# tungphambasement/DCNN

Hardware: AMD Instinct MI355X
Metric: images/sec (whole node) ResNet-18 Tiny-ImageNet training at 1/2/4/8 MI355X (higher is better)
Workload: dtype bf16; 1 GPU; model=resnet18_tiny_imagenet, global_batch=256, per_gpu_batch=256, parallelism=dp1, optimizer=adam, hipgraph=True, engine=native (C++ host API)

## Files before the change

### dcnn_amd/csrc/host/dcnn/ops.hpp

```cpp
#pragma once
#include <cstdint>

namespace dcnn {

struct ConvShape {
  int N, C, H, W, Co, KH, KW, SH, SW, PH, PW, OH, OW;
};
struct PoolShape {
  int N, C, H, W, OH, OW, KH, KW, SH, SW, PH, PW;
};
enum ActKind { ACT_RELU = 0, ACT_LEAKY_RELU = 1, ACT_ELU = 2, ACT_SIGMOID = 3, ACT_TANH = 4, ACT_LINEAR = 5 };

namespace cpu_ops {
void conv_fwd(const float* x, const float* w, const float* b, float* y, const ConvShape& s);
void conv_bwd(const float* x, const float* w, const float* dy, float* dx, float* dw, float* db, const ConvShape& s);
void dwconv_fwd(const float* x, const float* w, const float* b, float* y, const ConvShape& s);
void dwconv_bwd(const float* x, const float* w, const float* dy, float* dx, float* dw, float* db, const ConvShape& s);
void gconv_fwd(const float* x, const float* w, const float* b, float* y, const ConvShape& s, int groups);
void gconv_bwd(const float* x, const float* w, const float* dy, float* dx, float* dw, float* db, const ConvShape& s,
               int groups);
void dense_fwd(const float* x, const float* w, const float* b, float* y, long N, long In, long Out);
void dense_bwd(const float* x, const float* w, const float* dy, float* dx, float* dw, float* db, long N, long In,
               long Out);
void bn_fwd(const float* x, float* y, long N, long C, long HW, const float* g, const float* b, float eps, bool train,
// ... 14 lines not shown
void groupnorm_bwd(const float* x, const float* dy, const float* mean, const float* istd, const float* g, float* dx,
                   float* dg, float* db, long N, long C, long HW, long G);
void softmax_fwd(const float* x, float* y, long N, long C, long HW);
void softmax_bwd(const float* y, const float* dy, float* dx, long N, long C, long HW);
void dropout(const float* x, float* y, long n, float p, uint64_t seed);
void add(const float* a, const float* b, float* y, long n, bool relu);
void relu_mask(const float* dy, const float* y, float* dx, long n);
void adam(float* p, const float* g, float* m, float* v, long n, float lr, float b1, float b2, float eps, float bc1,
          float bc2, float wd, bool decoupled);
void sgd(float* p, const float* g, float* vel, long n, float lr, float momentum);
}

namespace gpu_ops {
void begin_deferred_reduce();
void end_deferred_reduce();
void flush_deferred_reduce();
void set_fault(int f);
void input_to_nhwc(const float* x, void* y, int N, int C, int HW);
void nhwc_to_nchw(const void* x, void* y, int N, int HW, int C);
void nchw_to_nhwc_bf16(const void* x, void* y, int N, int HW, int C);
void cast_bf16(const float* x, void* y, long n);
void zero(void* p, long nbytes);
const float* conv_fwd(const void* x, const void* w, const float* bias, void* y, const ConvShape& s,
                      int* stat_rows = nullptr);
struct BnbOperands {
  const void* y;
  const void* x;
  const float* mean;
  const float* istd;
  const float* gamma = nullptr;
  const float* beta = nullptr;
  bool mask_from_x = false;
};
const float* conv_dgrad(const void* dy, const void* w, void* dx, const ConvShape& s, const void* residual = nullptr,
                        bool w_transposed = false, const BnbOperands* bnb = nullptr, int* bnb_rows = nullptr);
void weight_transpose(const void* w, void* wt, int Co, int T, int C);
void multi_weight_transpose(const int64_t* table, int n, long max_tiles);
void conv_wgrad(const void* dy, const void* x, float* gw, float* gb, const ConvShape& s);
void dwconv_fwd(const void* x, const void* w, const float* bias, void* y, const ConvShape& s);
void dwconv_dgrad(const void* dy, const void* w, void* dx, const ConvShape& s, const void* residual = nullptr);
void dwconv_wgrad(const void* dy, const void* x, float* gw, float* gb, const ConvShape& s);
void gconv_fwd(const void* x, const void* w, const float* bias, void* y, const ConvShape& s, int groups);
void gconv_dgrad(const void* dy, const void* w, void* dx, const ConvShape& s, int groups,
                 const void* residual = nullptr);
void gconv_wgrad(const void* dy, const void* x, float* gw, float* gb, const ConvShape& s, int groups);
bool stem_ok(const ConvShape& s);
const float* stem_fwd(const float* x, const void* w, const float* bias, void* y, const ConvShape& s,
                      int* stat_rows = nullptr);
void stem_wgrad(const void* dy, const float* x, float* gw, float* gb, const ConvShape& s);
struct StemBn {
  const void* x;
  const float* mean;
  const float* istd;
// ... 93 lines not shown
```

### dcnn_amd/csrc/host/dist.cpp

```cpp
#include "dcnn/dist.hpp"

#include <arpa/inet.h>
#include <netdb.h>
#include <netinet/in.h>
#include <netinet/tcp.h>
#include <poll.h>
#include <sys/socket.h>
#include <unistd.h>

#include <cerrno>
#include <chrono>
#include <cstdlib>
#include <cstring>
#include <stdexcept>
#include <thread>

#include <algorithm>
#include <cstdint>

#include "../kernels/collective.h"
#include "dcnn/nn.hpp"
#include "dcnn/ops.hpp"

namespace dcnn {
// ... 414 lines not shown
    }
    if (!flow_) flow_ = gpu::flow_create();
    if (!ev_) ev_ = gpu::event_create();
  }
  reduced_lo_ = n_;
  next_ = lo_.size();
  nb_ = 0;
  model.set_backward_hook([this](size_t i) { on_layer_done(i); });
}

void DataParallel::reduce_layers(size_t lo_layer, size_t hi_layer) {
  if (comm_) {
    size_t lo = SIZE_MAX;
    for (size_t j = lo_layer; j < hi_layer; ++j) lo = std::min(lo, lo_[j]);
    if (lo == SIZE_MAX || lo >= reduced_lo_) return;
    gpu_ops::flush_deferred_reduce();
    gpu::event_record(ev_);
    gpu::flow_wait(flow_, ev_);
    comm_->all_reduce(g_ + lo, g_ + lo, reduced_lo_ - lo, 0, 4, flow_);
    reduced_lo_ = lo;
    ++nb_;
    return;
  }
  size_t total = 0;
  for (size_t j = lo_layer; j < hi_layer; ++j) total += layer_elems_[j];
  if (total == 0) return;
  pack_.resize(total);
  size_t o = 0;
  for (size_t j = lo_layer; j < hi_layer; ++j)
    for (const auto& s : segs_[j]) {
      std::memcpy(pack_.data() + o, s.first, s.second * 4);
// ... 2 lines not shown
  all_reduce_mean(pack_.data(), total);
  o = 0;
  for (size_t j = lo_layer; j < hi_layer; ++j)
    for (const auto& s : segs_[j]) {
      std::memcpy(s.first, pack_.data() + o, s.second * 4);
      o += s.second;
    }
  ++nb_;
}

void DataParallel::on_layer_done(size_t layer) {
  if (lo_.empty() || layer >= next_) return;
  size_t pending = 0;
  for (size_t j = layer; j < next_; ++j) pending += layer_elems_[j];
  if (pending == 0 || pending < bucket_elems_) return;
  reduce_layers(layer, next_);
  next_ = layer;
}

void DataParallel::finish() {
  if (lo_.empty()) throw std::runtime_error("DataParallel::finish: attach() first");
  if (next_ > 0) reduce_layers(0, next_);
  if (comm_) {
    gpu::event_record(ev_, flow_);
    gpu::flow_wait(gpu::flow(), ev_);
  }
  nb_last_ = nb_;
  nb_ = 0;
  reduced_lo_ = n_;
  next_ = lo_.size();
}

P2PLink::P2PLink(const std::string& unique_id, int rank, bool sender, int device) : sender_(sender) {
  if (!coll::available()) throw std::runtime_error("dist: RCCL unavailable: " + coll::load_error());
  if (rank != 0 && rank != 1) throw std::invalid_argument("P2PLink: rank 0 or 1");
  gpu::set_device(device);
  peer_ = 1 - rank;
// ... 92 lines not shown
```

### dcnn_amd/csrc/host/nn.cpp

```cpp
#include "dcnn/nn.hpp"

#include "../kernels/fusion_plan.h"

#include <algorithm>
#include <chrono>
#include <cmath>
#include <cstdio>
#include <cstdlib>
#include <filesystem>
#include <fstream>
#include <iostream>
#include <sstream>
#include <stdexcept>

namespace dcnn {

namespace {
struct Rng {
  uint64_t s;
  explicit Rng(uint64_t seed) : s(seed * 0x9e3779b97f4a7c15ull + 0x632be59bd9b4e019ull) {}
  uint64_t next() {
    uint64_t z = (s += 0x9e3779b97f4a7c15ull);
    z = (z ^ (z >> 30)) * 0xbf58476d1ce4e5b9ull;
    z = (z ^ (z >> 27)) * 0x94d049bb133111ebull;
// ... 157 lines not shown
  const Tensor& x_ = mbc().a;
  const ConvShape s = shape_for(x_.shape());
  gpu_ops::stem_wgrad_bn(dy.data(), x_.ptr<float>(), params_[0].grad.ptr<float>(),
                         bias_ ? params_[1].grad.ptr<float>() : nullptr, s, bn);
}

Tensor Conv2D::backward(const Tensor& dy) {
  const Tensor& x_ = mbc().a;
  const ConvShape s = shape_for(x_.shape());
  float* gb = bias_ ? params_[1].grad.ptr<float>() : nullptr;
  if (dev_.is_gpu() && x_.dtype() == DType::F32) {
    gpu_ops::stem_wgrad(dy.data(), x_.ptr<float>(), params_[0].grad.ptr<float>(), gb, s);
    return Tensor();
  }
  if (dev_.is_gpu()) {
    gpu_ops::conv_wgrad(dy.data(), x_.data(), params_[0].grad.ptr<float>(), gb, s);
    if (!input_grad_) return Tensor();
    Tensor dx = act_empty(x_.shape(), dev_);
    bool tr = false;
    const void* w = dgrad_operand(tr);
    if (bnb_from_ != nullptr) {
      const gpu_ops::BnbOperands ops = bnb_from_->bnb_operands(mb_);
      int rows = 0;
      const float* st = gpu_ops::conv_dgrad(dy.data(), w, dx.data(), s, nullptr, tr, &ops, &rows);
      if (rows > 0) bnb_from_->offer_bwd_stats(dx.data(), st, rows);
      return dx;
    }
    gpu_ops::conv_dgrad(dy.data(), w, dx.data(), s, nullptr, tr);
    return dx;
  }
  Tensor dx = act_empty(x_.shape(), dev_);
  {
    cpu_ops::conv_bwd(x_.ptr<float>(), params_[0].value.ptr<float>(), dy.ptr<float>(), dx.ptr<float>(),
                      params_[0].grad.ptr<float>(), gb, s);
  }
  return dx;
}

Tensor Conv2D::backward_residual(const Tensor& dy, const Tensor& residual) {
  const Tensor& x_ = mbc().a;
  if (!dev_.is_gpu() || x_.dtype() == DType::F32 || residual.shape() != x_.shape())
    throw std::runtime_error(name_ + ": backward_residual is a GPU fusion");
  const ConvShape s = shape_for(x_.shape());
  float* gb = bias_ ? params_[1].grad.ptr<float>() : nullptr;
  gpu_ops::conv_wgrad(dy.data(), x_.data(), params_[0].grad.ptr<float>(), gb, s);
  Tensor dx = act_empty(x_.shape(), dev_);
  bool tr = false;
  const void* w = dgrad_operand(tr);
  if (bnb_block_from_ != nullptr) {
    const gpu_ops::BnbOperands ops = bnb_block_from_->bnb_operands(mb_);
    int rows = 0;
    const float* st = gpu_ops::conv_dgrad(dy.data(), w, dx.data(), s, residual.data(), tr, &ops, &rows);
    if (rows > 0) bnb_block_from_->offer_bwd_stats(dx.data(), st, rows);
    return dx;
  }
  gpu_ops::conv_dgrad(dy.data(), w, dx.data(), s, residual.data(), tr);
  return dx;
}

DepthwiseConv2D::DepthwiseConv2D(int channels, int kh, int kw, int sh, int sw, int ph, int pw, bool bias,
// ... 1825 lines not shown
```

### dcnn_amd/csrc/host/ops_gpu.hip

```cpp
#include <hip/hip_runtime.h>

#include <algorithm>
#include <cmath>
#include <cstdio>
#include <cstdlib>
#include <cstring>
#include <map>
#include <mutex>
#include <stdexcept>
#include <string>
#include <unordered_map>
#include <vector>

#include "../kernels/api.h"
#include "dcnn/ops.hpp"
#include "dcnn/tensor.hpp"

#define HOST_HIP_CHECK(x)                                                                    \
  do {                                                                                       \
    hipError_t e_ = (x);                                                                     \
    if (e_ != hipSuccess) throw std::runtime_error(std::string(#x) + ": " + hipGetErrorString(e_)); \
  } while (0)

namespace dcnn {
// ... 444 lines not shown

void wgrad_reduce(const Tensor& hold, const Tensor& bhold, const float* slab, float* gw, long n, const float* bslab,
                  float* gb, long nb, int splits) {
  if (g_defer) {
    g_pending.push_back({hold, gw, n, splits});
    if (gb) g_pending.push_back({bhold, gb, nb, splits});
    g_pending_bytes += (size_t)n * splits * 4 + (gb ? (size_t)nb * splits * 4 : 0);
    if (reduce_flush_bytes() && g_pending_bytes >= reduce_flush_bytes()) launch_pending();
    return;
  }
  if (gb)
    splitk_reduce2(slab, gw, n, bslab, gb, nb, splits, 1, cur());
  else
    splitk_reduce(slab, gw, n, splits, 1, cur());
}
}

void begin_deferred_reduce() { g_defer = true; }
void set_fault(int f) { g_fault = f; }
void flush_deferred_reduce() {
  const bool on = g_defer;
  end_deferred_reduce();
  g_defer = on;
}
void end_deferred_reduce() {
  launch_pending();
  g_defer = false;
}

namespace {
void launch_pending() {
  for (size_t b = 0; b < g_pending.size(); b += kMaxRed) {
    MultiRed t{};
    t.count = (int)std::min(g_pending.size() - b, (size_t)kMaxRed);
    for (int k = 0; k < t.count; ++k) {
      const PendingRed& e = g_pending[b + k];
      t.e[k].slab = e.slab.ptr<float>();
      t.e[k].out = e.out;
      t.e[k].n = e.n;
      t.e[k].splits = e.splits;
    }
    multi_splitk_reduce(t, cur());
  }
  g_pending.clear();
  g_pending_bytes = 0;
}
// ... 164 lines not shown
      if (bnb && all_taps) {
        a.bnb = ba;
        a.stats = slab_of(gemm_g2_stat_rows(a.M, s.C));
      }
      gemm_g2(a, cur());
      return a.stats;
    }
  }
  NtArgs a{static_cast<const bf16*>(dy), wt, dx, s.N * s.H * s.W, s.C, K, 0, K, s.C, kConvDgrad, s.N, s.OH, s.OW,
           s.Co, s.H, s.W, s.KH, s.KW, s.SH, s.SW, s.PH, s.PW, nullptr, static_cast<const bf16*>(residual), nullptr,
           0, 0};
  gemm_nt(a, cur());
  return nullptr;
}

void conv_wgrad(const void* dy, const void* x, float* gw, float* gb, const ConvShape& s) {
  const int Ng = s.KH * s.KW * s.C, P = s.N * s.OH * s.OW;
  const long dyb = (long)P * s.Co * 2, xb = (long)s.N * s.H * s.W * s.C * 2;
  const int route = conv_wgrad_route(route_geom(s, -1));
  rec("wgrad", s, route, {{"bias", gb != nullptr}, {"deferred", g_defer}});
  if (route == ROUTE_HALO) {
    const int splits = hwgrad_splits(s.N, s.H, s.W, s.C, s.Co);
    Tensor hold, bhold;
    float* slab = wgrad_slab(SLAB, (size_t)splits * s.Co * Ng * 4, hold);
    float* bslab = gb ? wgrad_slab(BSLAB, (size_t)splits * s.Co * 4, bhold) : nullptr;
    HWArgs a{};
    a.dY = static_cast<const bf16*>(dy); a.X = static_cast<const bf16*>(x); a.slab = slab; a.bias_slab = bslab;
    a.dy_bytes = (unsigned)dyb; a.x_bytes = (unsigned)xb;
    a.NB = s.N; a.H = s.H; a.W = s.W; a.Cs = s.C; a.Co = s.Co; a.ntaps = 9;
    for (int t = 0; t < 9; ++t) { a.tap_dy[t] = t / 3 - 1; a.tap_dx[t] = t % 3 - 1; }
// ... 431 lines not shown
```

### dcnn_amd/csrc/kernels/api.h

```cpp
#pragma once
#include <hip/hip_runtime.h>
#include <stdint.h>

#include "fusion_plan.h"
typedef __bf16 bf16;

namespace dcnn {
struct BnbArgs {
  const bf16* y; const bf16* x; const float* mean; const float* istd;
  const float* gamma; const float* beta; int mask_x;
};
struct NtArgs {
  const bf16* A; const bf16* B; void* C;
  int M, N, K; int lda, ldb, ldc; int mode;
  int nb, sh, sw, cs, gh, gw; int kh, kw, strh, strw, padh, padw;
  const float* bias; const bf16* residual; float* stats; int out_f32; int relu;
};
struct TnArgs {
  const bf16* dY; const bf16* X; float* slab; float* bias_slab;
  int M, N, P; int mode; int nb, sh, sw, cs, gh, gw; int kh, kw, strh, strw, padh, padw; int ldx; int k_per_split;
};
struct G2Args {
  const bf16* A; const bf16* B; bf16* C;
  unsigned a_bytes, b_bytes;
// ... 63 lines not shown
void hconv3_enable(int on);
void hconv3_set_grid_cap(int n);
void hconv3_set_stamps(uintptr_t p);
struct HWArgs {
  const bf16* dY; const bf16* X; float* slab; float* bias_slab;
  unsigned dy_bytes, x_bytes;
  int NB, H, W, Cs, Co, ntaps;
  int tap_dy[9], tap_dx[9];
  int TH, TW, IMG, HPR, tiles_per_split;
  int ldy, ldx, npairs;
  int pair_yoff[3], pair_xoff[3], pair_bias[3];
};
void hwgrad(HWArgs a, int splits, hipStream_t s);
bool hwgrad_supported(int NB, int H, int W, int Cs, int Co, int ntaps);
int hwgrad_splits(int NB, int H, int W, int Cs, int Co);
bool hwgrad_f32_supported(int NB, int H, int W, int Cs, int Co);
int hwgrad_f32_splits(int NB, int H, int W, int Cs, int Co);
void hwgrad_f32(HWArgs a, int splits, hipStream_t s);
void hwgrad_set_version(int v);
bool hwgrad_s2_supported(int NB, int H, int W, int Cs, int Co);
int hwgrad_s2_splits(int NB, int H, int W, int Cs, int Co);
void hwgrad_s2(HWArgs a, int splits, hipStream_t s);

void gemm_nt(const NtArgs& a, hipStream_t s);
void gemm_g2(const G2Args& a, hipStream_t s);
void gemm_g2_set_splitk(int on);
int gemm_g2_splitk_enabled();
int gemm_g2_stat_rows(int M, int N);
int gemm_g2_row_tile(int M, int N);
void gemm_t2(T2Args a, int splits, hipStream_t s);
// ... 159 lines not shown
```

### dcnn_amd/csrc/kernels/bindings.cpp

```cpp
#include <tuple>
#include <pybind11/pybind11.h>
#include <pybind11/stl.h>
#include <algorithm>
#include <array>
#include <vector>
#include <hip/hip_runtime.h>
#include <stdint.h>

namespace py = pybind11;
#include "api.h"


using namespace dcnn;
void bind_runtime(py::module_& m);
void bind_rccl(py::module_& m);
template <typename T>
static inline T P(uintptr_t x) { return reinterpret_cast<T>(x); }
static inline hipStream_t S(uintptr_t x) { return reinterpret_cast<hipStream_t>(x); }

static void bind_gemm_g2(uintptr_t A, uintptr_t B, uintptr_t C, unsigned a_bytes, unsigned b_bytes, int M, int N, int Cs,
                         int H, int W, int GH, int GW, int SY, int SX, std::vector<std::array<int, 4>> taps, int ldb,
                         int ldc, int OH, int OW, int OSY, int OSX, int ORY, int ORX, uintptr_t bias, uintptr_t residual,
                         uintptr_t stats, int relu, uintptr_t zero_ptr, int zero_n, std::array<uintptr_t, 4> bnb,
                         uintptr_t stream, std::vector<std::array<int, 4>> classes = {}) {
// ... 129 lines not shown
          HWArgs a{};
          if (pairs.size() > 3) throw std::runtime_error("hwgrad: at most 3 operand pairs");
          a.npairs = (int)pairs.size(); a.ldy = ldy; a.ldx = ldx;
          for (size_t q = 0; q < pairs.size(); ++q) {
            a.pair_yoff[q] = pairs[q][0]; a.pair_xoff[q] = pairs[q][1]; a.pair_bias[q] = pairs[q][2];
          }
          a.dY = P<const bf16*>(dY); a.X = P<const bf16*>(X); a.slab = P<float*>(slab);
          a.bias_slab = P<float*>(bias_slab);
          a.dy_bytes = dy_bytes; a.x_bytes = x_bytes;
          a.NB = NB; a.H = H; a.W = W; a.Cs = Cs; a.Co = Co;
          if (taps.size() > 9 || taps.empty()) throw std::runtime_error("hwgrad: 1..9 taps");
          a.ntaps = (int)taps.size();
          for (size_t i = 0; i < taps.size(); ++i) { a.tap_dy[i] = taps[i][0]; a.tap_dx[i] = taps[i][1]; }
          hwgrad(a, splits, S(stream));
        });
  m.def("hwgrad_supported", &hwgrad_supported);
  m.def("hwgrad_s2_supported", &hwgrad_s2_supported);
  m.def("hwgrad_s2_splits", &hwgrad_s2_splits);
  m.def("hwgrad_s2",
        [](uintptr_t dY, uintptr_t X, uintptr_t slab, uintptr_t bias_slab, unsigned dy_bytes, unsigned x_bytes, int NB,
           int H, int W, int Cs, int Co, int splits, uintptr_t stream) {
          HWArgs a{};
          a.dY = P<const bf16*>(dY); a.X = P<const bf16*>(X); a.slab = P<float*>(slab);
          a.bias_slab = P<float*>(bias_slab);
          a.dy_bytes = dy_bytes; a.x_bytes = x_bytes;
          a.NB = NB; a.H = H; a.W = W; a.Cs = Cs; a.Co = Co; a.ntaps = 9;
          hwgrad_s2(a, splits, S(stream));
        });
  m.def("hwgrad_f32",
        [](uintptr_t dY, uintptr_t X, uintptr_t slab, uintptr_t bias_slab, unsigned dy_bytes, unsigned x_bytes, int NB,
// ... 447 lines not shown
```

### dcnn_amd/csrc/kernels/hwgrad.hip

```cpp
#include <type_traits>

#include "common.h"
#include "api.h"

namespace dcnn {

namespace {
constexpr unsigned kOOBw = 0x80000000u;
constexpr int PT = 128;

__device__ __forceinline__ void glds16w(i32x4 rsrc, char* lds, unsigned voff) { glds16_opaque(rsrc, lds, voff); }

__device__ __forceinline__ int xcd_remap_w(int bid, int nwg) {
  const int xcd = bid & 7, q = nwg >> 3, r = nwg & 7;
  const int base = xcd < r ? xcd * (q + 1) : r * (q + 1) + (xcd - r) * q;
  return base + (bid >> 3);
}

__device__ __forceinline__ int wswz(int row) { return (((row >> 1) & 1) | (((row >> 3) & 1) << 1)) << 1; }

__device__ __forceinline__ bf16x4 tr4(const char* base, int row, int col) {
  const int chn = col >> 3, within = (col & 7) * 2;
  const char* addr = base + row * 128 + ((chn ^ wswz(row)) << 4) + within;
  return __builtin_amdgcn_ds_read_tr16_b64_v4bf16((__attribute__((address_space(3))) bf16x4*)(const_cast<char*>(addr)));
// ... 204 lines not shown
  static_assert(TPX * IMG == PT, "tile must hold 128 pixels");
};

template <int K, int N, class F>
__device__ __forceinline__ void h3w_static_for(F&& f) {
  if constexpr (K < N) {
    f(std::integral_constant<int, K>{});
    h3w_static_for<K + 1, N>(f);
  }
}

__device__ __forceinline__ bf16x4 tr4_at(const char* addr) {
  return __builtin_amdgcn_ds_read_tr16_b64_v4bf16((__attribute__((address_space(3))) bf16x4*)(const_cast<char*>(addr)));
}

template <int TW, int TH, int IMG, int NS, int TSP = 1, bool F32 = false, bool C32 = false>
__global__ void __launch_bounds__(256 * TSP, 1) hwgrad2_kernel(HWArgs p) {
  prefetch_kernargs<sizeof(HWArgs)>();
  using G = HWGeo2<TW, TH, IMG>;
  constexpr int HNI = G::HNI, HW2P = G::HW2P, HPIP = G::HPIP, HPP = G::HPP, TPX = G::TPX, STAGE = G::STAGE;
  constexpr int INS = 4 + HNI;
  static_assert(NS == 2 || NS == 3, "2 or 3 stages");
  extern __shared__ __attribute__((aligned(16))) char smem[];
  const int tid = threadIdx.x, lane = tid & 63, wid = (tid >> 6) & 3, th = tid >> 8;
  constexpr int NT = 256 * TSP;
  const int co_tiles = p.Co / 64, ci_chunks = (p.Cs + 63) / 64;
  const int per_split = co_tiles * ci_chunks;
  const int lt = xcd_remap_w(blockIdx.x, gridDim.x);
  const int split = lt / per_split, rem = lt - split * per_split;
  const int pair = blockIdx.y, nsplits = gridDim.x / per_split;
  const int yoff = p.pair_yoff[pair], xoff = p.pair_xoff[pair];
  const int co0 = (rem / ci_chunks) * 64, c0 = (rem % ci_chunks) * 64;

  const int tx_tiles = p.W / TW, ty_tiles = p.H / TH, tpi = tx_tiles * ty_tiles;
  const int total_tiles = (p.NB / IMG) * tpi;
  const int tbeg = split * p.tiles_per_split;
  const int tend = min(total_tiles, tbeg + p.tiles_per_split);
  const i32x4 rsY = raw_rsrc(p.dY, p.dy_bytes);
  const i32x4 rsX = raw_rsrc(p.X, p.x_bytes);

  const int slot = lane & 7;
  unsigned y_rel[4], y_col[4];
#pragma unroll
  for (int i = 0; i < 4; ++i) {
    const int row = (wid * 4 + i) * 8 + (lane >> 3);
    const int im = row / TPX, r2 = row - im * TPX;
    y_rel[i] = (unsigned)((im * p.H + r2 / TW) * p.W + r2 % TW);
    y_col[i] = (unsigned)((yoff + co0 + ((slot ^ wswz2(row)) * 8)) * 2);
  }
  int h_rel[HNI], h_hy[HNI], h_hx[HNI];
#pragma unroll
  for (int j = 0; j < HNI; ++j) {
    const int row = (wid * HNI + j) * 8 + (lane >> 3);
    const int im = row / HPIP, r2 = row - im * HPIP;
// ... 63 lines not shown
        fb[k0][d] = PT * 128 + row * 128 + (((fci >> 2) ^ wswz2(row)) << 4) + (fci & 3) * 4;
      }
    }
  }
  auto blk_rows = [](int b) constexpr {
    if (TW == 16) return b * HW2P;
    if (TW == 8) return (b / 4) * HPIP + (b % 4) * 2 * HW2P;
    return b * HPIP;
  };

  auto run_f32 = [&](auto tb_c, auto ntw_c) {
    constexpr int TB = decltype(tb_c)::value, NTW = decltype(ntw_c)::value;
    f32x4 acc[NTW];
#pragma unroll
    for (int t = 0; t < NTW; ++t) acc[t] = f32x4{0.f, 0.f, 0.f, 0.f};
    const bool do_bias = p.bias_slab != nullptr && c0 == 0 && th == 0;
    float bias_acc = 0.f;
    if (NS == 3 && nt > 1)
      asm volatile("s_waitcnt vmcnt(%0)" ::"n"(INS) : "memory");
    else
      asm volatile("s_waitcnt vmcnt(0)" ::: "memory");
    __syncthreads();
    int cur = 0;
    for (int it = 0; it < nt; ++it) {
      if (it + NS - 1 < nt) load_tile(cur == 0 ? NS - 1 : cur - 1, tbeg + it + NS - 1);
      const char* S0 = smem + cur * STAGE;
      auto lds_f = [&](int off) { return *reinterpret_cast<const float*>(S0 + off); };
      float a[2], b[2][NTW];
      auto rd = [&](auto blk_c, int k0, int c) {
        constexpr int B = decltype(blk_c)::value;
        a[c] = lds_f(fa[k0] + B * 16 * 128);
// ... 17 lines not shown
      });
      if (do_bias) {
        const int col = tid & 31;
        for (int r = tid >> 5; r < PT; r += 8)
          bias_acc += *reinterpret_cast<const float*>(S0 + r * 128 + (((col >> 2) ^ wswz2(r)) << 4) + (col & 3) * 4);
      }
      if (NS == 3 && it + 2 < nt)
        asm volatile("s_waitcnt vmcnt(%0)\n\ts_waitcnt lgkmcnt(0)\n\ts_barrier" ::"n"(INS) : "memory");
      else
        asm volatile("s_waitcnt vmcnt(0)\n\ts_waitcnt lgkmcnt(0)\n\ts_barrier" ::: "memory");
      cur = cur == NS - 1 ? 0 : cur + 1;
    }
    const int Cs = p.Cs / 2, Co = p.Co / 2, cof = co0 / 2, cif = c0 / 2;
    const long Ng = 9l * Cs;
    const long slab_idx = (long)pair * nsplits + split;
    float* out = p.slab + slab_idx * Co * Ng;
    float* stg = reinterpret_cast<float*>(smem);
    constexpr int ET = G::EPI_TAPS;
#pragma unroll
    for (int t0 = 0; t0 < 9; t0 += ET) {
      __syncthreads();
#pragma unroll
      for (int u = 0; u < ET; ++u) {
        const int tl = t0 + u - TB;
        if (t0 + u < 9 && tl >= 0 && tl < NTW) {
#pragma unroll
          for (int r = 0; r < 4; ++r)
            stg[(u * 32 + 16 * (wid >> 1) + (lane >> 4) * 4 + r) * 36 + 16 * (wid & 1) + (lane & 15)] = acc[tl][r];
        }
      }
      __syncthreads();
      const int nrows = (9 - t0 < ET ? 9 - t0 : ET) * 32;
      for (int q = tid; q < nrows * 8; q += NT) {
        const int row = q >> 3, c4 = (q & 7) * 4;
        const int u = row >> 5, co = cof + (row & 31);
        const float4 v = *reinterpret_cast<const float4*>(stg + row * 36 + c4);
        *reinterpret_cast<float4*>(out + (long)co * Ng + (t0 + u) * Cs + cif + c4) = v;
      }
    }
    if (p.bias_slab != nullptr && c0 == 0) {
      __syncthreads();
      if (tid < 256) stg[tid] = bias_acc;
      __syncthreads();
      if (tid < 32) {
        float sum = 0.f;
#pragma unroll
        for (int gi = 0; gi < 8; ++gi) sum += stg[gi * 32 + tid];
        p.bias_slab[slab_idx * Co + cof + tid] = p.pair_bias[pair] ? sum : 0.f;
      }
    }
  };
  auto run = [&](auto tb_c, auto ntw_c) {
    constexpr int TB = decltype(tb_c)::value, NTW = decltype(ntw_c)::value;
    f32x4 acc[4][NTW];
  #pragma unroll
    for (int i = 0; i < 4; ++i)
  #pragma unroll
      for (int t = 0; t < NTW; ++t) acc[i][t] = f32x4{0.f, 0.f, 0.f, 0.f};

    const bool do_bias = p.bias_slab != nullptr && c0 == 0 && th == 0;
    float bias_acc = 0.f;
    if (NS == 3 && nt > 1)
      asm volatile("s_waitcnt vmcnt(%0)" ::"n"(INS) : "memory");
    else
      asm volatile("s_waitcnt vmcnt(0)" ::: "memory");
    __syncthreads();
    int cur = 0;
    for (int it = 0; it < nt; ++it) {
      if (it + NS - 1 < nt) load_tile(cur == 0 ? NS - 1 : cur - 1, tbeg + it + NS - 1);
      const char* S0 = smem + cur * STAGE;
      bf16x8 a[2][4], b[NTW];
      auto read_a = [&](int kk, bf16x8* av) {
  #pragma unroll
        for (int i = 0; i < 4; ++i) {
          const char* q = S0 + abase[i] + kk * 4096;
// ... 22 lines not shown
          if (kk + 1 < 4) b[t] = read_b(kk + 1, TB + t);
        }
      }
      if (do_bias) {
        const int col = tid & 63, chn = col >> 3, w = (col & 7) * 2;
        for (int r = wid; r < PT; r += 4)
          bias_acc += (float)*reinterpret_cast<const bf16*>(S0 + r * 128 + ((chn ^ wswz2(r)) << 4) + w);
      }
      if (NS == 3 && it + 2 < nt)
        asm volatile("s_waitcnt vmcnt(%0)\n\ts_waitcnt lgkmcnt(0)\n\ts_barrier" ::"n"(INS) : "memory");
      else
        asm volatile("s_waitcnt vmcnt(0)\n\ts_waitcnt lgkmcnt(0)\n\ts_barrier" ::: "memory");
      cur = cur == NS - 1 ? 0 : cur + 1;
    }

    const long Ng = 9l * p.Cs;
    const long slab_idx = (long)pair * nsplits + split;
    float* out = p.slab + slab_idx * p.Co * Ng;
    float* stg = reinterpret_cast<float*>(smem);
    constexpr int ET = G::EPI_TAPS;
  #pragma unroll
    for (int t0 = 0; t0 < 9; t0 += ET) {
      __syncthreads();
  #pragma unroll
      for (int u = 0; u < ET; ++u) {
        const int tl = t0 + u - TB;
        if (t0 + u < 9 && tl >= 0 && tl < NTW) {
  #pragma unroll
          for (int i = 0; i < 4; ++i)
  #pragma unroll
            for (int r = 0; r < 4; ++r)
              stg[(u * 64 + i * 16 + (lane >> 4) * 4 + r) * 68 + wid * 16 + (lane & 15)] = acc[i][tl][r];
        }
      }
      __syncthreads();
      const int nrows = (9 - t0 < ET ? 9 - t0 : ET) * 64;
      for (int q = tid; q < nrows * 16; q += NT) {
        const int row = q >> 4, c4 = (q & 15) * 4;
        const int u = row >> 6, co = co0 + (row & 63);
        const float4 v = *reinterpret_cast<const float4*>(stg + row * 68 + c4);
        if (!C32 || c0 + c4 < p.Cs) *reinterpret_cast<float4*>(out + (long)co * Ng + (t0 + u) * p.Cs + c0 + c4) = v;
      }
    }
    if (p.bias_slab != nullptr && c0 == 0) {
      __syncthreads();
      if (tid < 256) stg[tid] = bias_acc;
      __syncthreads();
      if (tid < 64)
        p.bias_slab[slab_idx * p.Co + co0 + tid] =
            p.pair_bias[pair] ? stg[tid] + stg[tid + 64] + stg[tid + 128] + stg[tid + 192] : 0.f;
    }

  };
  if constexpr (F32) {
    static_assert(TSP == 2, "fp32: 8 waves");
    if (th == 0) run_f32(std::integral_constant<int, 0>{}, std::integral_constant<int, 5>{});
    else run_f32(std::integral_constant<int, 5>{}, std::integral_constant<int, 4>{});
  } else if constexpr (TSP == 1) {
    run(std::integral_constant<int, 0>{}, std::integral_constant<int, 9>{});
  } else if constexpr (TSP == 2) {
    if (th == 0) run(std::integral_constant<int, 0>{}, std::integral_constant<int, 5>{});
    else run(std::integral_constant<int, 5>{}, std::integral_constant<int, 4>{});
  } else {
    if (th == 0) run(std::integral_constant<int, 0>{}, std::integral_constant<int, 3>{});
    else if (th == 1) run(std::integral_constant<int, 3>{}, std::integral_constant<int, 3>{});
    else run(std::integral_constant<int, 6>{}, std::integral_constant<int, 3>{});
  }
// ... 90 lines not shown
    DCNN_HIP_CHECK(hipFuncSetAttribute((const void*)k, hipFuncAttributeMaxDynamicSharedMemorySize, lds)); \
    hipLaunchKernelGGL(k, dim3(grid, a.npairs), dim3(256), lds, s, a);                                  \
    DCNN_LAUNCH_CHECK();                                                                                \
    return;                                                                                             \
  }
  DCNN_HW(16, 8, 1, 3)
  DCNN_HW(8, 8, 2, 3)
  DCNN_HW(4, 4, 8, 3)
  DCNN_HW(16, 8, 1, 2)
  DCNN_HW(8, 8, 2, 2)
  DCNN_HW(4, 4, 8, 2)
#undef DCNN_HW
  throw std::runtime_error("hwgrad: no kernel for this geometry");
}

bool hwgrad_f32_supported(int NB, int H, int W, int Cs, int Co) {
  int th, tw, img;
  if (Cs % 32 || Co % 32) return false;
  if (!hw_geometry(H, W, &th, &tw, &img) || NB % img) return false;
  return (long)NB * H * W * (Cs > Co ? Cs : Co) * 4 < (1l << 31);
}

int hwgrad_f32_splits(int NB, int H, int W, int Cs, int Co) { return hwgrad_splits(NB, H, W, 2 * Cs, 2 * Co); }

void hwgrad_f32(HWArgs a, int splits, hipStream_t s) {
  if (!hwgrad_f32_supported(a.NB, a.H, a.W, a.Cs, a.Co) || a.ntaps != 9)
    throw std::runtime_error("hwgrad_f32: unsupported shape");
  for (int t = 0; t < 9; ++t)
    if (a.tap_dy[t] != t / 3 - 1 || a.tap_dx[t] != t % 3 - 1) throw std::runtime_error("hwgrad_f32: 3x3 pad-1 taps only");
  if (splits != hwgrad_f32_splits(a.NB, a.H, a.W, a.Cs, a.Co)) throw std::runtime_error("hwgrad_f32: split count mismatch");
// ... 264 lines not shown
```

Before: 92160 images/sec.

## Group same-shape 3x3 weight-gradient convolutions into one multi-problem hwgrad launch

New measurement: 92480 images/sec (median of 6 runs). Within noise of the previous version (+0.4%).

```diff
diff --git a/dcnn_amd/csrc/host/dcnn/ops.hpp b/dcnn_amd/csrc/host/dcnn/ops.hpp
--- a/dcnn_amd/csrc/host/dcnn/ops.hpp
+++ b/dcnn_amd/csrc/host/dcnn/ops.hpp
@@ -2,6 +2,8 @@
 #include <cstdint>
 
 namespace dcnn {
+
+class Tensor;
 
 struct ConvShape {
   int N, C, H, W, Co, KH, KW, SH, SW, PH, PW, OH, OW;
@@ -52,7 +54,8 @@
 namespace gpu_ops {
 void begin_deferred_reduce();
 void end_deferred_reduce();
-void flush_deferred_reduce();
+void flush_deferred_reduce(bool keep_group = false);
+const float* pending_wgrad_end();
 void set_fault(int f);
 void input_to_nhwc(const float* x, void* y, int N, int C, int HW);
 void nhwc_to_nchw(const void* x, void* y, int N, int HW, int C);
@@ -75,6 +78,7 @@
 void weight_transpose(const void* w, void* wt, int Co, int T, int C);
 void multi_weight_transpose(const int64_t* table, int n, long max_tiles);
 void conv_wgrad(const void* dy, const void* x, float* gw, float* gb, const ConvShape& s);
+void conv_wgrad(const Tensor& dy, const Tensor& x, float* gw, float* gb, const ConvShape& s);
 void dwconv_fwd(const void* x, const void* w, const float* bias, void* y, const ConvShape& s);
 void dwconv_dgrad(const void* dy, const void* w, void* dx, const ConvShape& s, const void* residual = nullptr);
 void dwconv_wgrad(const void* dy, const void* x, float* gw, float* gb, const ConvShape& s);
diff --git a/dcnn_amd/csrc/host/dist.cpp b/dcnn_amd/csrc/host/dist.cpp
--- a/dcnn_amd/csrc/host/dist.cpp
+++ b/dcnn_amd/csrc/host/dist.cpp
@@ -452,7 +452,10 @@
     size_t lo = SIZE_MAX;
     for (size_t j = lo_layer; j < hi_layer; ++j) lo = std::min(lo, lo_[j]);
     if (lo == SIZE_MAX || lo >= reduced_lo_) return;
-    gpu_ops::flush_deferred_reduce();
+    if (const float* hi = gpu_ops::pending_wgrad_end())
+      if (hi > g_ + lo && hi <= g_ + n_) lo = (size_t)(hi - g_);
+    if (lo >= reduced_lo_) return;
+    gpu_ops::flush_deferred_reduce(true);
     gpu::event_record(ev_);
     gpu::flow_wait(flow_, ev_);
     comm_->all_reduce(g_ + lo, g_ + lo, reduced_lo_ - lo, 0, 4, flow_);
@@ -485,13 +488,23 @@
   size_t pending = 0;
   for (size_t j = layer; j < next_; ++j) pending += layer_elems_[j];
   if (pending == 0 || pending < bucket_elems_) return;
+  if (comm_) {
+    size_t lo = SIZE_MAX;
+    for (size_t j = layer; j < next_; ++j) lo = std::min(lo, lo_[j]);
+    const float* hi = gpu_ops::pending_wgrad_end();
+    if (lo != SIZE_MAX && hi && hi > g_ + lo && hi <= g_ + n_) {
+      const size_t start = (size_t)(hi - g_);
+      if (start >= reduced_lo_ || reduced_lo_ - start < bucket_elems_) return;
+    }
+  }
   reduce_layers(layer, next_);
   next_ = layer;
 }
 
 void DataParallel::finish() {
   if (lo_.empty()) throw std::runtime_error("DataParallel::finish: attach() first");
-  if (next_ > 0) reduce_layers(0, next_);
+  if (comm_) reduce_layers(0, lo_.size());
+  else if (next_ > 0) reduce_layers(0, next_);
   if (comm_) {
     gpu::event_record(ev_, flow_);
     gpu::flow_wait(gpu::flow(), ev_);
diff --git a/dcnn_amd/csrc/host/nn.cpp b/dcnn_amd/csrc/host/nn.cpp
--- a/dcnn_amd/csrc/host/nn.cpp
+++ b/dcnn_amd/csrc/host/nn.cpp
@@ -195,7 +195,7 @@
     return Tensor();
   }
   if (dev_.is_gpu()) {
-    gpu_ops::conv_wgrad(dy.data(), x_.data(), params_[0].grad.ptr<float>(), gb, s);
+    gpu_ops::conv_wgrad(dy, x_, params_[0].grad.ptr<float>(), gb, s);
     if (!input_grad_) return Tensor();
     Tensor dx = act_empty(x_.shape(), dev_);
     bool tr = false;
@@ -224,7 +224,7 @@
     throw std::runtime_error(name_ + ": backward_residual is a GPU fusion");
   const ConvShape s = shape_for(x_.shape());
   float* gb = bias_ ? params_[1].grad.ptr<float>() : nullptr;
-  gpu_ops::conv_wgrad(dy.data(), x_.data(), params_[0].grad.ptr<float>(), gb, s);
+  gpu_ops::conv_wgrad(dy, x_, params_[0].grad.ptr<float>(), gb, s);
   Tensor dx = act_empty(x_.shape(), dev_);
   bool tr = false;
   const void* w = dgrad_operand(tr);
diff --git a/dcnn_amd/csrc/host/ops_gpu.hip b/dcnn_amd/csrc/host/ops_gpu.hip
--- a/dcnn_amd/csrc/host/ops_gpu.hip
+++ b/dcnn_amd/csrc/host/ops_gpu.hip
@@ -482,22 +482,86 @@
   else
     splitk_reduce(slab, gw, n, splits, 1, cur());
 }
+
+struct PendingWgrad {
+  Tensor dy, x;
+  float* gw;
+  float* gb;
+  ConvShape s;
+};
+std::vector<PendingWgrad> g_wgroup;
+int wgrad_group_env() {
+  static const int mode = [] {
+    const char* v = std::getenv("DCNN_WGRAD_GROUP");
+    return v && v[0] >= '0' && v[0] <= '2' ? v[0] - '0' : 1;
+  }();
+  return mode;
+}
+void flush_wgrad_group() {
+  if (g_wgroup.empty()) return;
+  std::vector<PendingWgrad> q;
+  q.swap(g_wgroup);
+  const ConvShape& s = q[0].s;
+  const int P = (int)q.size(), Ng = 9 * s.C;
+  const bool serial = wgrad_group_env() != 2;
+  const int splits = serial ? hwgrad_splits(s.N, s.H, s.W, s.C, s.Co) : hwgrad_group_splits(s.N, s.H, s.W, s.C, s.Co, P);
+  HWGroupArgs a{};
+  a.nprob = P; a.serial = serial;
+  a.dy_bytes = (unsigned)((long)s.N * s.H * s.W * s.Co * 2); a.x_bytes = (unsigned)((long)s.N * s.H * s.W * s.C * 2);
+  a.NB = s.N; a.H = s.H; a.W = s.W; a.Cs = s.C; a.Co = s.Co; a.ntaps = 9;
+  for (int t = 0; t < 9; ++t) { a.tap_dy[t] = t / 3 - 1; a.tap_dx[t] = t % 3 - 1; }
+  Tensor hold[kHwGroupMax], bhold[kHwGroupMax];
+  for (int k = 0; k < P; ++k) {
+    a.g_dY[k] = static_cast<const bf16*>(q[k].dy.data()); a.g_X[k] = static_cast<const bf16*>(q[k].x.data());
+    a.g_slab[k] = wgrad_slab(SLAB, (size_t)splits * s.Co * Ng * 4, hold[k]);
+    a.g_bias_slab[k] = q[k].gb ? wgrad_slab(BSLAB, (size_t)splits * s.Co * 4, bhold[k]) : nullptr;
+  }
+  hwgrad_group(a, splits, cur());
+  for (int k = 0; k < P; ++k)
+    wgrad_reduce(hold[k], bhold[k], a.g_slab[k], q[k].gw, (long)s.Co * Ng, a.g_bias_slab[k], q[k].gb, s.Co, splits);
+}
 }
 
 void begin_deferred_reduce() { g_defer = true; }
 void set_fault(int f) { g_fault = f; }
-void flush_deferred_reduce() {
+void flush_deferred_reduce(bool keep_group) {
+  if (keep_group) {
+    launch_pending();
+    return;
+  }
   const bool on = g_defer;
   end_deferred_reduce();
   g_defer = on;
 }
+const float* pending_wgrad_end() {
+  const float* hi = nullptr;
+  for (const PendingWgrad& e : g_wgroup) {
+    hi = std::max(hi, static_cast<const float*>(e.gw + (long)e.s.Co * 9 * e.s.C));
+    if (e.gb) hi = std::max(hi, static_cast<const float*>(e.gb + e.s.Co));
+  }
+  return hi;
+}
 void end_deferred_reduce() {
+  flush_wgrad_group();
   launch_pending();
   g_defer = false;
 }
 
 namespace {
 void launch_pending() {
+  static const bool trace = [] {
+    const char* v = std::getenv("DCNN_TRACE_REDUCE");
+    return v && v[0] == '1';
+  }();
+  if (trace && !g_pending.empty()) {
+    size_t bytes = 0;
+    std::fprintf(stderr, "reduce:");
+    for (const PendingRed& e : g_pending) {
+      bytes += (size_t)e.n * e.splits * 4;
+      std::fprintf(stderr, " %dx%ld", e.splits, e.n);
+    }
+    std::fprintf(stderr, " | %zu slabs, %zu bytes of partials\n", g_pending.size(), bytes);
+  }
   for (size_t b = 0; b < g_pending.size(); b += kMaxRed) {
     MultiRed t{};
     t.count = (int)std::min(g_pending.size() - b, (size_t)kMaxRed);
@@ -692,6 +756,20 @@
   return nullptr;
 }
 
+void conv_wgrad(const Tensor& dy, const Tensor& x, float* gw, float* gb, const ConvShape& s) {
+  if (g_defer && wgrad_group_env() && conv_wgrad_route(route_geom(s, -1)) == ROUTE_HALO) {
+    rec("wgrad", s, ROUTE_HALO, {{"bias", gb != nullptr}, {"deferred", g_defer}});
+    if (!g_wgroup.empty()) {
+      const ConvShape& h = g_wgroup[0].s;
+      if (h.N != s.N || h.H != s.H || h.W != s.W || h.C != s.C || h.Co != s.Co) flush_wgrad_group();
+    }
+    g_wgroup.push_back({dy, x, gw, gb, s});
+    if ((int)g_wgroup.size() == kHwGroupMax) flush_wgrad_group();
+    return;
+  }
+  conv_wgrad(dy.data(), x.data(), gw, gb, s);
+}
+
 void conv_wgrad(const void* dy, const void* x, float* gw, float* gb, const ConvShape& s) {
   const int Ng = s.KH * s.KW * s.C, P = s.N * s.OH * s.OW;
   const long dyb = (long)P * s.Co * 2, xb = (long)s.N * s.H * s.W * s.C * 2;
diff --git a/dcnn_amd/csrc/kernels/api.h b/dcnn_amd/csrc/kernels/api.h
--- a/dcnn_amd/csrc/kernels/api.h
+++ b/dcnn_amd/csrc/kernels/api.h
@@ -101,6 +101,14 @@
 void hwgrad(HWArgs a, int splits, hipStream_t s);
 bool hwgrad_supported(int NB, int H, int W, int Cs, int Co, int ntaps);
 int hwgrad_splits(int NB, int H, int W, int Cs, int Co);
+constexpr int kHwGroupMax = 4;
+struct HWGroupArgs : HWArgs {
+  const bf16* g_dY[kHwGroupMax]; const bf16* g_X[kHwGroupMax];
+  float* g_slab[kHwGroupMax]; float* g_bias_slab[kHwGroupMax];
+  int nprob, serial;
+};
+int hwgrad_group_splits(int NB, int H, int W, int Cs, int Co, int nprob);
+void hwgrad_group(HWGroupArgs a, int splits, hipStream_t s);
 bool hwgrad_f32_supported(int NB, int H, int W, int Cs, int Co);
 int hwgrad_f32_splits(int NB, int H, int W, int Cs, int Co);
 void hwgrad_f32(HWArgs a, int splits, hipStream_t s);
diff --git a/dcnn_amd/csrc/kernels/bindings.cpp b/dcnn_amd/csrc/kernels/bindings.cpp
--- a/dcnn_amd/csrc/kernels/bindings.cpp
+++ b/dcnn_amd/csrc/kernels/bindings.cpp
@@ -167,6 +167,28 @@
           for (size_t i = 0; i < taps.size(); ++i) { a.tap_dy[i] = taps[i][0]; a.tap_dx[i] = taps[i][1]; }
           hwgrad(a, splits, S(stream));
         });
+  m.def("hwgrad_group",
+        [](std::vector<uintptr_t> dY, std::vector<uintptr_t> X, std::vector<uintptr_t> slab,
+           std::vector<uintptr_t> bias_slab, unsigned dy_bytes, unsigned x_bytes, int NB, int H, int W, int Cs, int Co,
+           int nprob, int splits, uintptr_t stream, int serial) {
+          if (nprob < 1 || nprob > kHwGroupMax || (int)dY.size() != nprob || (int)X.size() != nprob ||
+              (int)slab.size() != nprob || (int)bias_slab.size() != nprob)
+            throw std::runtime_error("hwgrad_group: 1..4 problems, one pointer of each kind per problem");
+          HWGroupArgs a{};
+          for (int q = 0; q < nprob; ++q) {
+            a.g_dY[q] = P<const bf16*>(dY[q]); a.g_X[q] = P<const bf16*>(X[q]);
+            a.g_slab[q] = P<float*>(slab[q]); a.g_bias_slab[q] = P<float*>(bias_slab[q]);
+          }
+          a.nprob = nprob; a.serial = serial;
+          a.dy_bytes = dy_bytes; a.x_bytes = x_bytes;
+          a.NB = NB; a.H = H; a.W = W; a.Cs = Cs; a.Co = Co; a.ntaps = 9;
+          for (int t = 0; t < 9; ++t) { a.tap_dy[t] = t / 3 - 1; a.tap_dx[t] = t % 3 - 1; }
+          hwgrad_group(a, splits, S(stream));
+        },
+        py::arg("dY"), py::arg("X"), py::arg("slab"), py::arg("bias_slab"), py::arg("dy_bytes"), py::arg("x_bytes"),
+        py::arg("NB"), py::arg("H"), py::arg("W"), py::arg("Cs"), py::arg("Co"), py::arg("nprob"), py::arg("splits"),
+        py::arg("stream"), py::arg("serial") = 0);
+  m.def("hwgrad_group_splits", &hwgrad_group_splits);
   m.def("hwgrad_supported", &hwgrad_supported);
   m.def("hwgrad_s2_supported", &hwgrad_s2_supported);
   m.def("hwgrad_s2_splits", &hwgrad_s2_splits);
diff --git a/dcnn_amd/csrc/kernels/hwgrad.hip b/dcnn_amd/csrc/kernels/hwgrad.hip
--- a/dcnn_amd/csrc/kernels/hwgrad.hip
+++ b/dcnn_amd/csrc/kernels/hwgrad.hip
@@ -242,9 +242,10 @@
   return __builtin_amdgcn_ds_read_tr16_b64_v4bf16((__attribute__((address_space(3))) bf16x4*)(const_cast<char*>(addr)));
 }
 
-template <int TW, int TH, int IMG, int NS, int TSP = 1, bool F32 = false, bool C32 = false>
-__global__ void __launch_bounds__(256 * TSP, 1) hwgrad2_kernel(HWArgs p) {
-  prefetch_kernargs<sizeof(HWArgs)>();
+template <int TW, int TH, int IMG, int NS, int TSP = 1, bool F32 = false, bool C32 = false, bool GRP = false>
+__global__ void __launch_bounds__(256 * TSP, 1) hwgrad2_kernel(std::conditional_t<GRP, HWGroupArgs, HWArgs> p) {
+  static_assert(!(GRP && F32), "groups: bf16 only");
+  prefetch_kernargs<sizeof(p)>();
   using G = HWGeo2<TW, TH, IMG>;
   constexpr int HNI = G::HNI, HW2P = G::HW2P, HPIP = G::HPIP, HPP = G::HPP, TPX = G::TPX, STAGE = G::STAGE;
   constexpr int INS = 4 + HNI;
@@ -254,9 +255,25 @@
   constexpr int NT = 256 * TSP;
   const int co_tiles = p.Co / 64, ci_chunks = (p.Cs + 63) / 64;
   const int per_split = co_tiles * ci_chunks;
-  const int lt = xcd_remap_w(blockIdx.x, gridDim.x);
+  int lt = xcd_remap_w(blockIdx.x, gridDim.x);
+  [[maybe_unused]] int prob = 0, prob_end = 1, wpp = 0;
+  if constexpr (GRP) {
+    if (p.serial) {
+      wpp = gridDim.x;
+      prob_end = p.nprob;
+    } else {
+      wpp = gridDim.x / p.nprob;
+      prob = lt / wpp;
+      lt -= prob * wpp;
+      prob_end = prob + 1;
+    }
+  }
+  auto dy_ptr = [&]() -> const bf16* { if constexpr (GRP) return p.g_dY[prob]; else return p.dY; };
+  auto x_ptr = [&]() -> const bf16* { if constexpr (GRP) return p.g_X[prob]; else return p.X; };
+  auto slab_ptr = [&]() -> float* { if constexpr (GRP) return p.g_slab[prob]; else return p.slab; };
+  auto bslab_ptr = [&]() -> float* { if constexpr (GRP) return p.g_bias_slab[prob]; else return p.bias_slab; };
   const int split = lt / per_split, rem = lt - split * per_split;
-  const int pair = blockIdx.y, nsplits = gridDim.x / per_split;
+  const int pair = blockIdx.y, nsplits = (GRP ? wpp : gridDim.x) / per_split;
   const int yoff = p.pair_yoff[pair], xoff = p.pair_xoff[pair];
   const int co0 = (rem / ci_chunks) * 64, c0 = (rem % ci_chunks) * 64;
 
@@ -264,8 +281,8 @@
   const int total_tiles = (p.NB / IMG) * tpi;
   const int tbeg = split * p.tiles_per_split;
   const int tend = min(total_tiles, tbeg + p.tiles_per_split);
-  const i32x4 rsY = raw_rsrc(p.dY, p.dy_bytes);
-  const i32x4 rsX = raw_rsrc(p.X, p.x_bytes);
+  i32x4 rsY = raw_rsrc(dy_ptr(), p.dy_bytes);
+  i32x4 rsX = raw_rsrc(x_ptr(), p.x_bytes);
 
   const int slot = lane & 7;
   unsigned y_rel[4], y_col[4];
@@ -359,7 +376,7 @@
     f32x4 acc[NTW];
 #pragma unroll
     for (int t = 0; t < NTW; ++t) acc[t] = f32x4{0.f, 0.f, 0.f, 0.f};
-    const bool do_bias = p.bias_slab != nullptr && c0 == 0 && th == 0;
+    const bool do_bias = bslab_ptr() != nullptr && c0 == 0 && th == 0;
     float bias_acc = 0.f;
     if (NS == 3 && nt > 1)
       asm volatile("s_waitcnt vmcnt(%0)" ::"n"(INS) : "memory");
@@ -407,7 +424,7 @@
     const int Cs = p.Cs / 2, Co = p.Co / 2, cof = co0 / 2, cif = c0 / 2;
     const long Ng = 9l * Cs;
     const long slab_idx = (long)pair * nsplits + split;
-    float* out = p.slab + slab_idx * Co * Ng;
+    float* out = slab_ptr() + slab_idx * Co * Ng;
     float* stg = reinterpret_cast<float*>(smem);
     constexpr int ET = G::EPI_TAPS;
 #pragma unroll
@@ -431,7 +448,7 @@
         *reinterpret_cast<float4*>(out + (long)co * Ng + (t0 + u) * Cs + cif + c4) = v;
       }
     }
-    if (p.bias_slab != nullptr && c0 == 0) {
+    if (bslab_ptr() != nullptr && c0 == 0) {
       __syncthreads();
       if (tid < 256) stg[tid] = bias_acc;
       __syncthreads();
@@ -439,19 +456,20 @@
         float sum = 0.f;
 #pragma unroll
         for (int gi = 0; gi < 8; ++gi) sum += stg[gi * 32 + tid];
-        p.bias_slab[slab_idx * Co + cof + tid] = p.pair_bias[pair] ? sum : 0.f;
+        bslab_ptr()[slab_idx * Co + cof + tid] = p.pair_bias[pair] ? sum : 0.f;
       }
     }
   };
   auto run = [&](auto tb_c, auto ntw_c) {
     constexpr int TB = decltype(tb_c)::value, NTW = decltype(ntw_c)::value;
     f32x4 acc[4][NTW];
+    for (;;) {
   #pragma unroll
     for (int i = 0; i < 4; ++i)
   #pragma unroll
       for (int t = 0; t < NTW; ++t) acc[i][t] = f32x4{0.f, 0.f, 0.f, 0.f};
 
-    const bool do_bias = p.bias_slab != nullptr && c0 == 0 && th == 0;
+    const bool do_bias = bslab_ptr() != nullptr && c0 == 0 && th == 0;
     float bias_acc = 0.f;
     if (NS == 3 && nt > 1)
       asm volatile("s_waitcnt vmcnt(%0)" ::"n"(INS) : "memory");
@@ -504,9 +522,11 @@
       cur = cur == NS - 1 ? 0 : cur + 1;
     }
 
+    int tid_e = tid, lane_e = lane;
+    if constexpr (GRP) asm volatile("" : "+v"(tid_e), "+v"(lane_e));
     const long Ng = 9l * p.Cs;
     const long slab_idx = (long)pair * nsplits + split;
-    float* out = p.slab + slab_idx * p.Co * Ng;
+    float* out = slab_ptr() + slab_idx * p.Co * Ng;
     float* stg = reinterpret_cast<float*>(smem);
     constexpr int ET = G::EPI_TAPS;
   #pragma unroll
@@ -520,27 +540,39 @@
           for (int i = 0; i < 4; ++i)
   #pragma unroll
             for (int r = 0; r < 4; ++r)
-              stg[(u * 64 + i * 16 + (lane >> 4) * 4 + r) * 68 + wid * 16 + (lane & 15)] = acc[i][tl][r];
+              stg[(u * 64 + i * 16 + (lane_e >> 4) * 4 + r) * 68 + wid * 16 + (lane_e & 15)] = acc[i][tl][r];
         }
       }
       __syncthreads();
       const int nrows = (9 - t0 < ET ? 9 - t0 : ET) * 64;
-      for (int q = tid; q < nrows * 16; q += NT) {
+      for (int q = tid_e; q < nrows * 16; q += NT) {
         const int row = q >> 4, c4 = (q & 15) * 4;
         const int u = row >> 6, co = co0 + (row & 63);
         const float4 v = *reinterpret_cast<const float4*>(stg + row * 68 + c4);
         if (!C32 || c0 + c4 < p.Cs) *reinterpret_cast<float4*>(out + (long)co * Ng + (t0 + u) * p.Cs + c0 + c4) = v;
       }
     }
-    if (p.bias_slab != nullptr && c0 == 0) {
+    if (bslab_ptr() != nullptr && c0 == 0) {
       __syncthreads();
-      if (tid < 256) stg[tid] = bias_acc;
+      if (tid_e < 256) stg[tid_e] = bias_acc;
       __syncthreads();
-      if (tid < 64)
-        p.bias_slab[slab_idx * p.Co + co0 + tid] =
-            p.pair_bias[pair] ? stg[tid] + stg[tid + 64] + stg[tid + 128] + stg[tid + 192] : 0.f;
-    }
-
+      if (tid_e < 64)
+        bslab_ptr()[slab_idx * p.Co + co0 + tid_e] =
+            p.pair_bias[pair] ? stg[tid_e] + stg[tid_e + 64] + stg[tid_e + 128] + stg[tid_e + 192] : 0.f;
+    }
+    if constexpr (!GRP) {
+      break;
+    } else {
+      if (++prob >= prob_end) break;
+      __syncthreads();
+      rsY = raw_rsrc(dy_ptr(), p.dy_bytes);
+      rsX = raw_rsrc(x_ptr(), p.x_bytes);
+      int tb = tbeg;
+      asm volatile("" : "+s"(tb));
+      if (nt > 0) load_tile(0, tb);
+      if (NS == 3 && nt > 1) load_tile(1, tb + 1);
+    }
+    }
   };
   if constexpr (F32) {
     static_assert(TSP == 2, "fp32: 8 waves");
@@ -661,6 +693,64 @@
   throw std::runtime_error("hwgrad: no kernel for this geometry");
 }
 
+int hwgrad_group_splits(int NB, int H, int W, int Cs, int Co, int nprob) {
+  int th, tw, img;
+  if (nprob <= 1 || g_hwgrad_version != 2 || !hw_geometry(H, W, &th, &tw, &img)) return hwgrad_splits(NB, H, W, Cs, Co);
+  const int total = (NB / img) * (H / th) * (W / tw);
+  const int per_split = (Co / 64) * ((Cs + 63) / 64);
+  int want = (kHwTargetBlocks / nprob) / per_split;
+  if (want < 1) want = 1;
+  if (want > total) want = total;
+  constexpr int min_tps = 2;
+  if (want > total / min_tps) want = total / min_tps > 1 ? total / min_tps : 1;
+  const int tps = (total + want - 1) / want;
+  return (total + tps - 1) / tps;
+}
+
+void hwgrad_group(HWGroupArgs a, int splits, hipStream_t s) {
+  if (a.nprob < 1 || a.nprob > kHwGroupMax) throw std::runtime_error("hwgrad_group: 1..4 problems");
+  if (a.npairs > 1) throw std::runtime_error("hwgrad_group: plain operands only");
+  if (splits != (a.serial ? hwgrad_splits(a.NB, a.H, a.W, a.Cs, a.Co)
+                          : hwgrad_group_splits(a.NB, a.H, a.W, a.Cs, a.Co, a.nprob)))
+    throw std::runtime_error("hwgrad_group: split count mismatch");
+  if (a.nprob == 1 || g_hwgrad_version != 2) {
+    for (int q = 0; q < a.nprob; ++q) {
+      HWArgs one = a;
+      one.dY = a.g_dY[q]; one.X = a.g_X[q]; one.slab = a.g_slab[q]; one.bias_slab = a.g_bias_slab[q];
+      hwgrad(one, splits, s);
+    }
+    return;
+  }
+  if (!hwgrad_supported(a.NB, a.H, a.W, a.Cs, a.Co, a.ntaps)) throw std::runtime_error("hwgrad_group: unsupported shape");
+  for (int t = 0; t < 9; ++t)
+    if (a.tap_dy[t] != t / 3 - 1 || a.tap_dx[t] != t % 3 - 1) throw std::runtime_error("hwgrad_group: 3x3 pad-1 taps only");
+  for (int q = 0; q < a.nprob; ++q)
+    if (!a.g_dY[q] || !a.g_X[q] || !a.g_slab[q]) throw std::runtime_error("hwgrad_group: null operand");
+  a.npairs = 1; a.ldy = a.Co; a.ldx = a.Cs;
+  a.pair_yoff[0] = a.pair_xoff[0] = 0; a.pair_bias[0] = 1;
+  a.dY = nullptr; a.X = nullptr; a.slab = nullptr; a.bias_slab = nullptr;
+  hw_geometry(a.H, a.W, &a.TH, &a.TW, &a.IMG);
+  const int total = (a.NB / a.IMG) * (a.H / a.TH) * (a.W / a.TW);
+  a.tiles_per_split = (total + splits - 1) / splits;
+  const int grid = (a.serial ? 1 : a.nprob) * splits * (a.Co / 64) * ((a.Cs + 63) / 64);
+  const bool c32 = a.Cs % 64 != 0;
+#define DCNN_HWG(TW_, TH_, IMG_, NS_)                                                                   \
+  if (a.TW == TW_ && a.TH == TH_ && a.IMG == IMG_) {                                                    \
+    auto k = c32 ? hwgrad2_kernel<TW_, TH_, IMG_, NS_, 2, false, true, true>                            \
+                 : hwgrad2_kernel<TW_, TH_, IMG_, NS_, 2, false, false, true>;                          \
+    const int lds = NS_ * HWGeo2<TW_, TH_, IMG_>::STAGE;                                                \
+    DCNN_HIP_CHECK(hipFuncSetAttribute((const void*)k, hipFuncAttributeMaxDynamicSharedMemorySize, lds)); \
+    hipLaunchKernelGGL(k, dim3(grid, 1), dim3(512), lds, s, a);                                         \
+    DCNN_LAUNCH_CHECK();                                                                                \
+    return;                                                                                             \
+  }
+  DCNN_HWG(16, 8, 1, 3)
+  DCNN_HWG(8, 8, 2, 2)
+  DCNN_HWG(4, 4, 8, 2)
+#undef DCNN_HWG
+  throw std::runtime_error("hwgrad_group: no kernel for this geometry");
+}
+
 bool hwgrad_f32_supported(int NB, int H, int W, int Cs, int Co) {
   int th, tw, img;
   if (Cs % 32 || Co % 32) return false;
```
